# Pixie8888/R3DFSSeg

Hardware: AMD Instinct MI355X
Metric: episodes/sec S3DIS 2-way 5-shot 2048-pt (MPTI+attention, train step: forward+backward+grad all-reduce+Adam) (higher is better)
Workload: dtype f32 (index-free GEMMs -- self-attention, 1x1 convolutions, weight gradients, the EdgeConv backward's edge GEMMs -- as bf16x3 split products on the bf16 MFMA with fp32 accumulate; every index-deciding result: fp32)

## Files before the change

### r3dfsseg_amd/csrc/head_graph.hip

```cpp
#include "common.h"

#define HG_NC 4
typedef unsigned short hg_col_t;
#define HG_ROWS_PER_BLOCK_MIN 4
#define HG_MAX_PART 2048

struct HgEp {
  long nodes, nbr, y, z, g, lam, dn;
  long desc;
  long ws;
  long stats;
  long labels, logits, loss, pred;
};
#define HG_WS(p) p = (decltype(p))((const char*)(p) + (long)ep * st.ws * 4)
#define HG_AT(p, stride) p += (long)ep * (stride)

__global__ __launch_bounds__(256) void r3d_graph_bits_kernel(const int* __restrict__ nbr, int kp1, const int* __restrict__ n_dev,
                                                             int n_cap, int words, unsigned* __restrict__ outb, HgEp st) {
  __shared__ unsigned bm[4][1024];
  const int ep = blockIdx.y;
  nbr += (long)ep * st.nbr * kp1; HG_AT(n_dev, st.desc); HG_WS(outb);
  const int n = min(*n_dev, n_cap);
  const int w = threadIdx.x >> 6, lane = threadIdx.x & 63;
  const int i = blockIdx.x * 4 + w;
// ... 630 lines not shown
  {
    const int ep = blockIdx.y;
    HG_AT(B, b_stride); HG_WS(dinv); HG_WS(agg); HG_WS(MW); HG_AT(n_dev, st.desc); HG_AT(x, x_stride); HG_WS(r); HG_WS(p); HG_WS(q);
    HG_WS(part); HG_WS(Einv); HG_WS(cg);
  }
  __shared__ float4 sm[4];
  __shared__ float4 rs[HG_UROWS];
  __shared__ float us[HG_UROWS];
  __shared__ int ag[HG_UROWS];
  __shared__ __attribute__((aligned(16))) float mu_s[HG_M * HG_NC];
  __shared__ float4 wpart[2 * 4 * HG_M];
  __shared__ double d_s[HG_M * HG_NC];
  __shared__ float t_s[HG_M * HG_NC];
  __shared__ float rr_s[HG_NC];
  __shared__ int last_s;
  __shared__ float tile_s[4 * 32 * 65];
  __shared__ float4 dot_s[HG_UROWS];
  const int row0 = blockIdx.x * HG_UROWS;
  float m[64];
  if (mode == 1) cg_load_mw_column(MW, row0, n_cap, m);
  const int n = min(*n_dev, n_cap);
  if (mode == 1) mu_s[threadIdx.x] = cg->mu[threadIdx.x];
  __syncthreads();
  if (mode == 1) {
    const int lane = threadIdx.x & 63, w = threadIdx.x >> 6;
    float* tl = tile_s + w * (32 * 65);
#pragma unroll
    for (int h = 0; h < 2; ++h) {
#pragma unroll
      for (int k = 0; k < 32; ++k) tl[k * 65 + lane] = m[32 * h + k];
      __builtin_amdgcn_wave_barrier();
      const int rk = lane & 31, a0 = 32 * (lane >> 5);
      float4 acc = f4_zero();
#pragma unroll 8
      for (int a = 0; a < 32; ++a) {
        const float mv = tl[rk * 65 + a0 + a];
        const float4 cv = *reinterpret_cast<const float4*>(&mu_s[(a0 + a) * HG_NC]);
        acc.x = __builtin_fmaf(mv, cv.x, acc.x); acc.y = __builtin_fmaf(mv, cv.y, acc.y);
        acc.z = __builtin_fmaf(mv, cv.z, acc.z); acc.w = __builtin_fmaf(mv, cv.w, acc.w);
      }
      acc.x += __shfl_xor(acc.x, 32); acc.y += __shfl_xor(acc.y, 32);
      acc.z += __shfl_xor(acc.z, 32); acc.w += __shfl_xor(acc.w, 32);
      if (lane < 32) dot_s[64 * w + 32 * h + lane] = acc;
      __builtin_amdgcn_wave_barrier();
    }
  }
  __syncthreads();
  {
    const int i = row0 + threadIdx.x;
    float4 rv = f4_zero();
    float u = 0.f;
    int a = 0;
    if (i < n) {
      u = 1.f / dinv[i];
      a = agg[i];
      rv = B[i];
      if (mode == 1) {
        const float4 s = dot_s[threadIdx.x];
        rv = make_float4(rv.x - s.x, rv.y - s.y, rv.z - s.z, rv.w - s.w);
        x[i] = make_float4(u * mu_s[a * HG_NC + 0], u * mu_s[a * HG_NC + 1], u * mu_s[a * HG_NC + 2], u * mu_s[a * HG_NC + 3]);
        r[i] = rv;
      }
    }
    if (mode == 1 && i < n_cap) {
      p[i] = f4_zero(); q[i] = f4_zero();
      if (i >= n) { x[i] = f4_zero(); r[i] = f4_zero(); }
    }
    rs[threadIdx.x] = rv; us[threadIdx.x] = u; ag[threadIdx.x] = a;
  }
  __syncthreads();
  cg_block_partials(rs, us, ag, row0, n, m, mode == 1, part + (long)blockIdx.x * HG_PART, sm, wpart);
  if (cg_delivered_last(cg, gridDim.x, &last_s)) cg_reduce_step(part, gridDim.x, Einv, mode, 0, tol2, cg, d_s, t_s, rr_s);
}

__global__ __launch_bounds__(256) void r3d_cg_spmv_kernel(
    const int* __restrict__ row_ptr, const hg_col_t* __restrict__ col, const float* __restrict__ val,
    const float* __restrict__ dinv, const int* __restrict__ agg, const float* __restrict__ MW,
    const int* __restrict__ n_dev, int n_cap, float alpha_lp, int it, int rows_per_block,
    const float4* __restrict__ r, float4* __restrict__ p, float4* __restrict__ q,
    float4* __restrict__ part_pq, const CgState* __restrict__ cg, HgEp st) {
  __shared__ float4 mu_s[HG_M];
  __shared__ float4 wsum[4];
  {
    const int ep = blockIdx.y;
    HG_WS(cg);
    if (cg->done) return;
    HG_WS(row_ptr); HG_WS(col); HG_WS(val); HG_WS(dinv); HG_WS(agg); HG_WS(MW); HG_AT(n_dev, st.desc); HG_WS(r); HG_WS(p);
    HG_WS(q); HG_WS(part_pq);
  }
  const int n = min(*n_dev, n_cap);
  const int lane = threadIdx.x & 63, w = threadIdx.x >> 6;
  if (threadIdx.x < HG_M) mu_s[threadIdx.x] = reinterpret_cast<const float4*>(cg->mu)[threadIdx.x];
  const float4 beta = *reinterpret_cast<const float4*>(cg->beta);
  __syncthreads();
  const float4 mul = mu_s[lane];
  float4 acc_pq = f4_zero();
  const int row0 = blockIdx.x * rows_per_block + w * (rows_per_block / 4);
  for (int rr_i = 0; rr_i < rows_per_block / 4; ++rr_i) {
    const int i = row0 + rr_i;
    if (i >= n) break;
    float4 s = f4_zero();
    const int rb = row_ptr[i], re = row_ptr[i + 1];
    const float mw = MW[(long)i * HG_M + lane];
    for (int e0 = rb + lane; e0 < re; e0 += 384) {
      int jv[6];
      float av[6];
#pragma unroll
      for (int u = 0; u < 6; ++u) {
        const int e = e0 + 64 * u;
        const int ec = min(e, re - 1);
        jv[u] = col[ec];
        av[u] = r3d_keep(val[ec], e < re);
      }
      float4 rj[6];
#pragma unroll
      for (int u = 0; u < 6; ++u) rj[u] = r[jv[u]];
#pragma unroll
      for (int u = 0; u < 6; ++u) {
        s.x = __builtin_fmaf(av[u], rj[u].x, s.x); s.y = __builtin_fmaf(av[u], rj[u].y, s.y);
        s.z = __builtin_fmaf(av[u], rj[u].z, s.z); s.w = __builtin_fmaf(av[u], rj[u].w, s.w);
      }
    }
    s.x = __builtin_fmaf(mw, mul.x, -alpha_lp * s.x); s.y = __builtin_fmaf(mw, mul.y, -alpha_lp * s.y);
    s.z = __builtin_fmaf(mw, mul.z, -alpha_lp * s.z); s.w = __builtin_fmaf(mw, mul.w, -alpha_lp * s.w);
#pragma unroll
    for (int o = 32; o > 0; o >>= 1) {
      s.x += __shfl_xor(s.x, o); s.y += __shfl_xor(s.y, o);
      s.z += __shfl_xor(s.z, o); s.w += __shfl_xor(s.w, o);
    }
    if (lane == 0) {
      const float4 ri = r[i], pi = p[i], qi = q[i];
      const float u = 1.f / dinv[i];
      const float4 m = mu_s[agg[i]];
      const float4 pn = make_float4((ri.x + u * m.x) + beta.x * pi.x, (ri.y + u * m.y) + beta.y * pi.y,
                                    (ri.z + u * m.z) + beta.z * pi.z, (ri.w + u * m.w) + beta.w * pi.w);
      const float4 qn = make_float4((ri.x + s.x) + beta.x * qi.x, (ri.y + s.y) + beta.y * qi.y,
                                    (ri.z + s.z) + beta.z * qi.z, (ri.w + s.w) + beta.w * qi.w);
      p[i] = pn;
      q[i] = qn;
      acc_pq.x += pn.x * qn.x; acc_pq.y += pn.y * qn.y; acc_pq.z += pn.z * qn.z; acc_pq.w += pn.w * qn.w;
    }
  }
  if (lane == 0) wsum[w] = acc_pq;
  __syncthreads();
  if (threadIdx.x == 0) {
    float4 t = wsum[0];
    for (int q2 = 1; q2 < 4; ++q2) { t.x += wsum[q2].x; t.y += wsum[q2].y; t.z += wsum[q2].z; t.w += wsum[q2].w; }
    part_pq[blockIdx.x] = t;
  }
}

#define SL_ROWS 128
#define SL_WAVES 8
#define SL_RPW (SL_ROWS / SL_WAVES)
#define SL_MAX_LDS (144 * 1024)
__global__ __launch_bounds__(64 * SL_WAVES) void r3d_cg_spmv_lds_kernel(
    const int* __restrict__ row_ptr, const hg_col_t* __restrict__ col, const float* __restrict__ val,
    const float* __restrict__ dinv, const int* __restrict__ agg, const float* __restrict__ MW,
    const int* __restrict__ n_dev, int n_cap, float alpha_lp, int it, int rows_per_block,
    const float4* __restrict__ r, float4* __restrict__ p, float4* __restrict__ q,
    float4* __restrict__ part_pq , const CgState* __restrict__ cg, HgEp st) {
  extern __shared__ __attribute__((aligned(16))) float4 rs[];
  __shared__ float4 mu_s[HG_M];
  {
    const int ep = blockIdx.y;
    HG_WS(cg);
    if (cg->done) return;
    HG_WS(row_ptr); HG_WS(col); HG_WS(val); HG_WS(dinv); HG_WS(agg); HG_WS(MW); HG_AT(n_dev, st.desc); HG_WS(r); HG_WS(p);
    HG_WS(q); HG_WS(part_pq);
  }
  __shared__ float4 pq_s[SL_ROWS];
  const int n = min(*n_dev, n_cap);
  const int tid = threadIdx.x, lane = tid & 63, w = tid >> 6;
  const int n_wg = gridDim.x, bx = blockIdx.x;
  const int n_part = (n_cap + 3) / 4;
  auto row_of = [&](int k) {
    const int l = SL_WAVES * k + w;
    return 4 * ((l >> 2) * n_wg + bx) + (l & 3);
  };
  int nrows = 0;
#pragma unroll
  for (int k = 0; k < SL_RPW; ++k) nrows += row_of(k) < n ? 1 : 0;
  const int my_row = min(row_of(min(lane, SL_RPW - 1)), max(n - 1, 0));
  const int my_rb = row_ptr[my_row], my_re = row_ptr[my_row + 1];
  for (int i0 = tid; i0 < n; i0 += 4 * 64 * SL_WAVES) {
    float4 v[4];
#pragma unroll
    for (int u = 0; u < 4; ++u) v[u] = r[min(i0 + u * 64 * SL_WAVES, n - 1)];
#pragma unroll
    for (int u = 0; u < 4; ++u)
      if (i0 + u * 64 * SL_WAVES < n) rs[i0 + u * 64 * SL_WAVES] = v[u];
  }
  if (tid < HG_M) mu_s[tid] = reinterpret_cast<const float4*>(cg->mu)[tid];
  const float4 beta = *reinterpret_cast<const float4*>(cg->beta);
  __syncthreads();
  const float4 mul = mu_s[lane];
  int jv[6], jn[6];
  float av[6], an[6];
  float mw = 0.f, mwn = 0.f;
  auto issue = [&](int k, int (&jj)[6], float (&aa)[6], float& mm) {
    const int rb = __builtin_amdgcn_readlane(my_rb, k), re = __builtin_amdgcn_readlane(my_re, k);
#pragma unroll
    for (int u = 0; u < 6; ++u) {
      const int e = rb + lane + 64 * u;
      const int ec = max(min(e, re - 1), 0);
      jj[u] = col[ec];
      aa[u] = r3d_keep(val[ec], e < re);
    }
    mm = MW[(long)row_of(k) * HG_M + lane];
  };
  float4 tot[2] = {f4_zero(), f4_zero()};
  if (nrows > 0) issue(0, jv, av, mw);
#pragma unroll
  for (int h = 0; h < 2; ++h) {
    float4 acc[8];
#pragma unroll
    for (int kk = 0; kk < 8; ++kk) {
      const int k = 8 * h + kk;
      acc[kk] = f4_zero();
      if (k < nrows) {
        if (k + 1 < nrows) issue(k + 1, jn, an, mwn);
        const int rb = __builtin_amdgcn_readlane(my_rb, k), re = __builtin_amdgcn_readlane(my_re, k);
        float4 s = f4_zero();
        {
          float4 rj[6];
#pragma unroll
          for (int u = 0; u < 6; ++u) rj[u] = rs[jv[u]];
#pragma unroll
          for (int u = 0; u < 6; ++u) {
            s.x = __builtin_fmaf(av[u], rj[u].x, s.x); s.y = __builtin_fmaf(av[u], rj[u].y, s.y);
            s.z = __builtin_fmaf(av[u], rj[u].z, s.z); s.w = __builtin_fmaf(av[u], rj[u].w, s.w);
          }
        }
        for (int e0 = rb + 384; e0 < re; e0 += 384) {
          int j2[6];
          float a2[6];
#pragma unroll
          for (int u = 0; u < 6; ++u) {
            const int e = e0 + lane + 64 * u;
            const int ec = min(e, re - 1);
            j2[u] = col[ec];
            a2[u] = r3d_keep(val[ec], e < re);
          }
#pragma unroll
          for (int u = 0; u < 6; ++u) {
            const float4 rj = rs[j2[u]];
            s.x = __builtin_fmaf(a2[u], rj.x, s.x); s.y = __builtin_fmaf(a2[u], rj.y, s.y);
            s.z = __builtin_fmaf(a2[u], rj.z, s.z); s.w = __builtin_fmaf(a2[u], rj.w, s.w);
          }
        }
        s.x = __builtin_fmaf(mw, mul.x, -alpha_lp * s.x); s.y = __builtin_fmaf(mw, mul.y, -alpha_lp * s.y);
        s.z = __builtin_fmaf(mw, mul.z, -alpha_lp * s.z); s.w = __builtin_fmaf(mw, mul.w, -alpha_lp * s.w);
        acc[kk] = s;
#pragma unroll
        for (int u = 0; u < 6; ++u) { jv[u] = jn[u]; av[u] = an[u]; }
        mw = mwn;
      }
    }
    float4 a4[4], a2[2], a1;
    {
      const bool hi = (lane & 32) != 0;
#pragma unroll
      for (int t = 0; t < 4; ++t) {
        const float4 keepv = hi ? acc[4 + t] : acc[t], sendv = hi ? acc[t] : acc[4 + t];
        a4[t].x = keepv.x + __shfl_xor(sendv.x, 32); a4[t].y = keepv.y + __shfl_xor(sendv.y, 32);
        a4[t].z = keepv.z + __shfl_xor(sendv.z, 32); a4[t].w = keepv.w + __shfl_xor(sendv.w, 32);
      }
    }
    {
      const bool hi = (lane & 16) != 0;
#pragma unroll
      for (int t = 0; t < 2; ++t) {
        const float4 keepv = hi ? a4[2 + t] : a4[t], sendv = hi ? a4[t] : a4[2 + t];
        a2[t].x = keepv.x + __shfl_xor(sendv.x, 16); a2[t].y = keepv.y + __shfl_xor(sendv.y, 16);
        a2[t].z = keepv.z + __shfl_xor(sendv.z, 16); a2[t].w = keepv.w + __shfl_xor(sendv.w, 16);
      }
    }
    {
      const bool hi = (lane & 8) != 0;
      const float4 keepv = hi ? a2[1] : a2[0], sendv = hi ? a2[0] : a2[1];
      a1.x = keepv.x + __shfl_xor(sendv.x, 8); a1.y = keepv.y + __shfl_xor(sendv.y, 8);
      a1.z = keepv.z + __shfl_xor(sendv.z, 8); a1.w = keepv.w + __shfl_xor(sendv.w, 8);
    }
#pragma unroll
    for (int o = 4; o > 0; o >>= 1) {
      a1.x += __shfl_xor(a1.x, o); a1.y += __shfl_xor(a1.y, o);
      a1.z += __shfl_xor(a1.z, o); a1.w += __shfl_xor(a1.w, o);
    }
    tot[h] = a1;
  }
  float4 acc_pq = f4_zero();
  const int trow = 8 * (lane & 7) + (lane >> 3);
  if ((lane & 7) < 2 && trow < nrows) {
    const float4 keep = (lane & 1) ? tot[1] : tot[0];
    const int i = row_of(trow);
    const float4 ri = rs[i], pi = p[i], qi = q[i];
    const float u = 1.f / dinv[i];
    const float4 m = mu_s[agg[i]];
    const float4 pn = make_float4((ri.x + u * m.x) + beta.x * pi.x, (ri.y + u * m.y) + beta.y * pi.y,
                                  (ri.z + u * m.z) + beta.z * pi.z, (ri.w + u * m.w) + beta.w * pi.w);
    const float4 qn = make_float4((ri.x + keep.x) + beta.x * qi.x, (ri.y + keep.y) + beta.y * qi.y,
                                  (ri.z + keep.z) + beta.z * qi.z, (ri.w + keep.w) + beta.w * qi.w);
    p[i] = pn;
    q[i] = qn;
    acc_pq = make_float4(pn.x * qn.x, pn.y * qn.y, pn.z * qn.z, pn.w * qn.w);
  }
  if ((lane & 7) < 2) pq_s[SL_WAVES * trow + w] = acc_pq;
  __syncthreads();
  if (tid < SL_ROWS / 4) {
    const float4 a = pq_s[4 * tid], b2 = pq_s[4 * tid + 1], c2 = pq_s[4 * tid + 2], d2 = pq_s[4 * tid + 3];
    const float4 t = make_float4(((a.x + b2.x) + c2.x) + d2.x, ((a.y + b2.y) + c2.y) + d2.y, ((a.z + b2.z) + c2.z) + d2.z,
                                 ((a.w + b2.w) + c2.w) + d2.w);
    const int gidx = tid * n_wg + bx;
    if (gidx < n_part) part_pq[gidx] = t;
  }
}

#ifdef CG_STAMPS
__device__ unsigned long long g_cg_dbg[32];
#define CSTAMP(i) do { if (it == 3 && threadIdx.x == 0 && blockIdx.x == 0) g_cg_dbg[i] = __builtin_amdgcn_s_memtime(); } while (0)
#define CSTAMP_LAST(i) do { if (it == 3 && threadIdx.x == 0) g_cg_dbg[16 + i] = __builtin_amdgcn_s_memtime(); } while (0)
extern "C" int r3d_cg_debug_read(unsigned long long* out32) {
  return hipMemcpyFromSymbol(out32, HIP_SYMBOL(g_cg_dbg), sizeof(g_cg_dbg)) == hipSuccess ? 0 : 1;
}
#else
#define CSTAMP(i)
#define CSTAMP_LAST(i)
#endif

__global__ __launch_bounds__(256) void r3d_cg_update_kernel(
    const int* __restrict__ n_dev, int n_cap, int it, int nblk_pq, const float* __restrict__ dinv, const int* __restrict__ agg,
    const float* __restrict__ MW, const float4* __restrict__ p, const float4* __restrict__ q, float4* __restrict__ x,
    float4* __restrict__ r, const float4* __restrict__ part_pq, float* __restrict__ part, const float* __restrict__ Einv,
    float tol2, CgState* __restrict__ cg, HgEp st, long x_stride) {
  __shared__ float4 sm[4];
  __shared__ float4 rs[HG_UROWS];
  __shared__ float us[HG_UROWS];
  __shared__ int ag[HG_UROWS];
  __shared__ float4 wpart[2 * 4 * HG_M];
  __shared__ double d_s[HG_M * HG_NC];
  __shared__ float t_s[HG_M * HG_NC];
  __shared__ float rr_s[HG_NC];
  __shared__ int last_s;
  {
    const int ep = blockIdx.y;
    HG_AT(n_dev, st.desc); HG_WS(dinv); HG_WS(agg); HG_WS(MW); HG_WS(p); HG_WS(q); HG_AT(x, x_stride); HG_WS(r); HG_WS(part_pq);
    HG_WS(part); HG_WS(Einv); HG_WS(cg);
  }
  const int row0 = blockIdx.x * HG_UROWS;
  const int i = row0 + threadIdx.x;
  const int ic = min(i, n_cap - 1);
  float m[64];
  CSTAMP(0);
  cg_load_mw_column(MW, row0, n_cap, m);
  const float4 pi = p[ic], qi = q[ic];
  float4 xi = x[ic], ri = r[ic];
  const float dv = dinv[ic];
  const int av = agg[ic];
  const int done = cg->done;
  const float4 rz = *reinterpret_cast<const float4*>(cg->rz);
  const int n = min(*n_dev, n_cap);
  const float4 pq = reduce_partials(part_pq, nblk_pq, sm);
  CSTAMP(1);
  if (done) return;
  float4 al;
  al.x = pq.x > 0.f ? rz.x / pq.x : 0.f;
  al.y = pq.y > 0.f ? rz.y / pq.y : 0.f;
  al.z = pq.z > 0.f ? rz.z / pq.z : 0.f;
  al.w = pq.w > 0.f ? rz.w / pq.w : 0.f;
  float u = 0.f;
  int a = 0;
  if (i < n) {
    xi.x += al.x * pi.x; xi.y += al.y * pi.y; xi.z += al.z * pi.z; xi.w += al.w * pi.w;
    ri.x -= al.x * qi.x; ri.y -= al.y * qi.y; ri.z -= al.z * qi.z; ri.w -= al.w * qi.w;
    x[i] = xi; r[i] = ri;
    u = 1.f / dv;
    a = av;
  } else {
    ri = f4_zero();
  }
  rs[threadIdx.x] = ri; us[threadIdx.x] = u; ag[threadIdx.x] = a;
  __syncthreads();
  CSTAMP(2);
  cg_block_partials(rs, us, ag, row0, n, m, true, part + (long)blockIdx.x * HG_PART, sm, wpart);
  CSTAMP(3);
  const bool last = cg_delivered_last(cg, gridDim.x, &last_s);
  CSTAMP(4);
  if (last) {
    CSTAMP_LAST(0);
    cg_reduce_step(part, gridDim.x, Einv, 1, it + 1, tol2, cg, d_s, t_s, rr_s);
    CSTAMP_LAST(1);
  }
}

__global__ __launch_bounds__(1024) void r3d_logits_ce_kernel(const float4* __restrict__ Z, const float4* __restrict__ Z2,
                                                             const int* __restrict__ desc_nproto, int n_q, int N, int n_classes,
                                                             const long long* __restrict__ labels,
                                                             float* __restrict__ logits ,
                                                             float* __restrict__ loss_out, int* __restrict__ pred_out, HgEp st) {
  __shared__ float red[16];
  {
    const int ep = blockIdx.x;
    HG_AT(Z, st.z); HG_AT(desc_nproto, st.desc); HG_AT(logits, st.logits);
    if (Z2) HG_AT(Z2, st.z);
    if (labels) HG_AT(labels, st.labels);
    if (loss_out) HG_AT(loss_out, st.loss);
    if (pred_out) HG_AT(pred_out, st.pred);
  }
  const int n_proto = *desc_nproto;
  float acc = 0.f;
  for (int e = threadIdx.x; e < n_q * N; e += blockDim.x) {
    const int qi = e / N, p = e - qi * N;
    const float4 z = Z[n_proto + e];
    const float4 z2 = Z2 ? Z2[n_proto + e] : f4_zero();
    const float zv[8] = {z.x, z.y, z.z, z.w, z2.x, z2.y, z2.z, z2.w};
    float mx = zv[0];
    int am = 0;
    for (int c = 1; c < n_classes; ++c) if (zv[c] > mx) { mx = zv[c]; am = c; }
    float se = 0.f;
    for (int c = 0; c < n_classes; ++c) {
      logits[((long)qi * n_classes + c) * N + p] = zv[c];
      se += expf(zv[c] - mx);
    }
    if (labels) {
      const int lab = (int)labels[e];
      acc += (mx + logf(se)) - zv[lab];
    }
    if (pred_out) pred_out[e] = am;
  }
  acc = r3d_wave_sum(acc);
  if ((threadIdx.x & 63) == 0) red[threadIdx.x >> 6] = acc;
  __syncthreads();
  if (threadIdx.x == 0) {
    float t = 0.f;
    for (int w = 0; w < (int)(blockDim.x >> 6); ++w) t += red[w];
    if (loss_out) *loss_out = t / (float)(n_q * N);
  }
}

struct LpWs {
  unsigned *outb, *sym;
  int *row_len, *row_ptr, *agg;
  hg_col_t* col;
  float *val, *dinv, *wdir, *MW, *Epart, *part;
  float* Einv;
  float4 *r, *p, *q, *part_pq;
  CgState* cg;
  long words, total;
};

static inline long hg_vblocks(int n_cap) { return r3d_cdiv(n_cap, HG_UROWS); }

static LpWs lp_carve(int32_t* ws, int n_cap, int kp1) {
  LpWs L;
  L.words = (n_cap + 31) / 32;
  const long nnz_cap = 2L * n_cap * (kp1 - 1);
  int32_t* wp = ws;
  auto align4 = [&]() { wp += (4 - ((wp - ws) & 3)) & 3; };
  L.outb = (unsigned*)wp; wp += n_cap * L.words;
  L.sym = (unsigned*)wp; wp += n_cap * L.words;
  L.row_len = wp; wp += n_cap + 8;
  L.row_ptr = wp; wp += n_cap + 8;
  L.col = (hg_col_t*)wp; wp += (nnz_cap + 1) / 2;
  L.val = (float*)wp; wp += nnz_cap;
  L.wdir = (float*)wp; wp += 2 * nnz_cap;
  L.dinv = (float*)wp; wp += n_cap;
  L.agg = wp; wp += n_cap;
  align4();
  L.MW = (float*)wp; wp += (long)n_cap * HG_M;
  L.Epart = (float*)wp; wp += (long)HG_EBLOCKS * HG_M * HG_M;
  align4();
  L.Einv = (float*)wp; wp += (long)HG_M * HG_M;
  L.part = (float*)wp; wp += hg_vblocks(n_cap) * HG_PART;
  align4();
  L.r = (float4*)wp; wp += 4L * n_cap;
  L.p = (float4*)wp; wp += 4L * n_cap;
  L.q = (float4*)wp; wp += 4L * n_cap;
  L.part_pq = (float4*)wp; wp += 4L * HG_MAX_PART;
  L.cg = (CgState*)wp; wp += (sizeof(CgState) + 3) / 4;
  L.total = (wp - ws) + 64;
  return L;
}

extern "C" long r3d_lp_ws_words(int n_cap, int kp1) { return lp_carve(nullptr, n_cap, kp1).total; }

extern "C" int r3d_lp_ws_offsets(int n_cap, int kp1, long* out6) {
  R3D_REQUIRE(out6 && n_cap > 0 && kp1 >= 2, "r3d_lp_ws_offsets: bad arguments");
  const LpWs L = lp_carve(nullptr, n_cap, kp1);
  const int32_t* base = nullptr;
  out6[0] = (const int32_t*)L.row_ptr - base; out6[1] = (const int32_t*)L.col - base; out6[2] = (const int32_t*)L.val - base;
  out6[3] = (const int32_t*)L.dinv - base; out6[4] = (const int32_t*)L.agg - base; out6[5] = (const int32_t*)L.cg - base;
  return R3D_OK;
}

__global__ void r3d_weights_compare_kernel(const int* __restrict__ row_ptr, const int* __restrict__ n_dev, int n_cap,
                                           const float* __restrict__ wdir, const float* __restrict__ wdir2, long scratch_stride,
                                           int* __restrict__ mismatch, HgEp st) {
  const int ep = blockIdx.y;
  HG_WS(row_ptr); HG_AT(n_dev, st.desc); HG_WS(wdir);
  wdir2 += (long)ep * scratch_stride;
  const int n = min(*n_dev, n_cap);
  const long nnz2 = 2L * row_ptr[n];
  int bad = 0;
  for (long e = (long)blockIdx.x * blockDim.x + threadIdx.x; e < nnz2; e += (long)gridDim.x * blockDim.x)
    bad += __float_as_uint(wdir[e]) != __float_as_uint(wdir2[e]) ? 1 : 0;
  bad = (int)r3d_wave_sum((float)bad);
  if ((threadIdx.x & 63) == 0 && bad) atomicAdd(mismatch, bad);
}
extern "C" long r3d_graph_weights_verify_words(int n_cap, int kp1) {
  const long nnz_cap = 2L * n_cap * (kp1 - 1);
  return 2 * nnz_cap + nnz_cap + n_cap + 64;
}
extern "C" int r3d_graph_weights_verify(int n_ep, const float* nodes, long ldn, int D, const int32_t* n_dev, long desc_stride,
                                        int n_cap, int kp1, float sigma, int32_t* ws, long ws_words, long ws_stride,
                                        float* scratch, int32_t* mismatch_out, void* stream) {
  R3D_REQUIRE(nodes && n_dev && ws && scratch && mismatch_out, "r3d_graph_weights_verify: null pointer");
  R3D_REQUIRE(n_cap > 0 && kp1 >= 2 && ws_words >= r3d_lp_ws_words(n_cap, kp1) && n_ep >= 1 &&
                  (n_ep == 1 || ((ws_stride & 3) == 0 && ws_stride >= ws_words)),
              "r3d_graph_weights_verify: bad arguments");
  hipStream_t st = (hipStream_t)stream;
  const LpWs L = lp_carve(ws, n_cap, kp1);
  const long nnz_cap = 2L * n_cap * (kp1 - 1), per = r3d_graph_weights_verify_words(n_cap, kp1);
  for (int e = 0; e < n_ep; ++e) {
    HgEp one{};
    float* base = scratch + (long)e * per;
    int32_t* wse = ws + (long)e * ws_stride;
    const LpWs Le = lp_carve(wse, n_cap, kp1);
    hipLaunchKernelGGL(r3d_graph_weights_kernel, dim3(n_cap, 1), dim3(256), 0, st, nodes + (long)e * n_cap * ldn, ldn, D, Le.outb,
                       (int)Le.words, n_dev + (long)e * desc_stride, n_cap, Le.row_ptr, Le.col, sigma, base + 2 * nnz_cap,
                       base + 3 * nnz_cap, base, one);
  }
  HgEp ep{};
  ep.desc = desc_stride; ep.ws = ws_stride;
  hipLaunchKernelGGL(r3d_weights_compare_kernel, dim3(256, n_ep), dim3(256), 0, st, L.row_ptr, n_dev, n_cap, L.wdir, scratch, per,
                     mismatch_out, ep);
  R3D_LAUNCH_CHECK("r3d_graph_weights_verify");
  return R3D_OK;
}

__global__ void r3d_cg_stats_kernel(const CgState* __restrict__ cg, int* __restrict__ stats_out, HgEp st) {
  const int ep = blockIdx.x;
  HG_WS(cg); HG_AT(stats_out, st.stats);
  if (threadIdx.x == 0) { stats_out[0] = cg->done; stats_out[1] = cg->iters; }
}

static int lp_coarse_space(const LpWs& L, const float* nodes, long ldn, int D, const int32_t* n_dev, const int32_t* n_proto_dev,
                           int n_cap, float alpha, int n_ep, const HgEp& ep, hipStream_t st) {
  const int agg_rpw = 4;
  const size_t agg_lds = ((size_t)HG_M * (D | 1) + 4 * D) * sizeof(float);
  static bool lds_opt_in = false;
  if (!lds_opt_in) {
    hipFuncSetAttribute((const void*)r3d_cg_aggregate_kernel, hipFuncAttributeMaxDynamicSharedMemorySize, 96 * 1024);
    lds_opt_in = true;
  }
  hipLaunchKernelGGL(r3d_cg_aggregate_kernel, dim3(r3d_cdiv(n_cap, 4 * agg_rpw), n_ep), dim3(256), agg_lds, st, nodes, ldn, D,
                     n_dev, n_proto_dev, n_cap, agg_rpw, L.agg, ep);
  hipLaunchKernelGGL(r3d_cg_mw_kernel, dim3(r3d_cdiv(n_cap, 4), n_ep), dim3(256), 0, st, L.row_ptr, L.col, L.val, L.dinv, L.agg,
                     n_dev, n_cap, alpha, 1, L.MW, ep);
  hipLaunchKernelGGL(r3d_cg_epart_kernel, dim3(HG_EBLOCKS, n_ep), dim3(128), 0, st, L.MW, L.dinv, L.agg, n_dev, n_cap, L.Epart,
                     ep);
  hipLaunchKernelGGL(r3d_cg_einv_kernel, dim3(n_ep), dim3(1024), 0, st, L.Epart, L.Einv, ep);
  return R3D_OK;
}

static int g_cg_lds_min_blocks = 256;
extern "C" int r3d_debug_set_cg_spmv_lds_min_blocks(int min_blocks) {
  const int old = g_cg_lds_min_blocks;
  g_cg_lds_min_blocks = min_blocks;
  return old;
}

static int lp_solve(const LpWs& L, const float* RHS, long rhs_stride, const int32_t* n_dev, int n_cap, float alpha, int max_iter,
                    float tol, float* X, long x_stride, int32_t* stats_out, int n_ep, const HgEp& ep, hipStream_t st) {
  const int nblk_v = (int)hg_vblocks(n_cap);
  int rpb = HG_ROWS_PER_BLOCK_MIN;
  while (r3d_cdiv(n_cap, rpb) > HG_MAX_PART) rpb += 4;
  const int nblk_s = r3d_cdiv(n_cap, rpb);
  R3D_REQUIRE(nblk_s <= HG_MAX_PART, "r3d_label_propagate: n_cap too large");
  float4* x = (float4*)X;
  const float tol2 = tol * tol;
  r3d_fill_words_ep(&L.cg->ticket, 0u, 1, n_ep, ep.ws, st);
  for (int mode = 0; mode < 2; ++mode)
    hipLaunchKernelGGL(r3d_cg_init_kernel, dim3(nblk_v, n_ep), dim3(256), 0, st, (const float4*)RHS, L.dinv, L.agg, L.MW, n_dev,
                       n_cap, mode, x, L.r, L.p, L.q, L.part, L.Einv, tol2, L.cg, ep, rhs_stride, x_stride);
  const size_t lds_r = (size_t)n_cap * sizeof(float4);
  const bool use_lds = lds_r <= SL_MAX_LDS && rpb == HG_ROWS_PER_BLOCK_MIN && (long)n_ep * r3d_cdiv(n_cap, SL_ROWS) >= g_cg_lds_min_blocks;
  if (use_lds) {
    static size_t attr = 0;
    if (lds_r > attr) {
      hipError_t e = hipFuncSetAttribute((const void*)r3d_cg_spmv_lds_kernel, hipFuncAttributeMaxDynamicSharedMemorySize, (int)lds_r);
      R3D_REQUIRE(e == hipSuccess, "r3d_label_propagate: cannot reserve %zu B of LDS: %s", lds_r, hipGetErrorString(e));
      attr = lds_r;
    }
  }
  const int nblk_l = r3d_cdiv(n_cap, SL_ROWS);
  const int nblk_pq = nblk_s;
  for (int it = 0; it < max_iter; ++it) {
    if (use_lds)
      hipLaunchKernelGGL(r3d_cg_spmv_lds_kernel, dim3(nblk_l, n_ep), dim3(64 * SL_WAVES), lds_r, st, L.row_ptr, L.col, L.val, L.dinv,
                         L.agg, L.MW, n_dev, n_cap, alpha, it, SL_ROWS, L.r, L.p, L.q, L.part_pq, L.cg, ep);
    else
      hipLaunchKernelGGL(r3d_cg_spmv_kernel, dim3(nblk_s, n_ep), dim3(256), 0, st, L.row_ptr, L.col, L.val, L.dinv, L.agg, L.MW,
                         n_dev, n_cap, alpha, it, rpb, L.r, L.p, L.q, L.part_pq, L.cg, ep);
    hipLaunchKernelGGL(r3d_cg_update_kernel, dim3(nblk_v, n_ep), dim3(256), 0, st, n_dev, n_cap, it, nblk_pq, L.dinv, L.agg, L.MW,
                       L.p, L.q, x, L.r, L.part_pq, L.part, L.Einv, tol2, L.cg, ep, x_stride);
  }
  if (stats_out) hipLaunchKernelGGL(r3d_cg_stats_kernel, dim3(n_ep), dim3(64), 0, st, L.cg, stats_out, ep);
  return R3D_OK;
}

static int label_propagate_impl(int n_ep, const HgEp& ep, const float* nodes, long ldn, int D, const int32_t* nbr, int kp1,
                                const float* Y, const int32_t* n_dev, const int32_t* n_proto_dev, int n_cap, float sigma,
                                float alpha, int max_iter, float tol, float* Z, int32_t* ws, long ws_words, int32_t* stats_out,
                                void* stream) {
  R3D_REQUIRE(nodes && nbr && Y && n_dev && n_proto_dev && Z && ws, "r3d_label_propagate: null pointer");
  R3D_REQUIRE(n_cap > 0 && kp1 >= 2 && ws_words >= r3d_lp_ws_words(n_cap, kp1),
              "r3d_label_propagate: workspace of %ld words, r3d_lp_ws_words(%d, %d) = %ld needed", ws_words, n_cap, kp1,
              n_cap > 0 && kp1 >= 2 ? r3d_lp_ws_words(n_cap, kp1) : -1L);
  R3D_REQUIRE((ldn & 3) == 0 && ((uintptr_t)nodes & 15) == 0,
              "r3d_label_propagate: node rows are read as float4: ldn must be a multiple of 4 and nodes 16-byte aligned");
  R3D_REQUIRE(n_cap > 0 && n_cap <= 32768 && D > 0 && D <= 256 && (D & 3) == 0 && kp1 >= 2,
              "r3d_label_propagate: unsupported n_cap=%d D=%d kp1=%d", n_cap, D, kp1);
  R3D_REQUIRE(max_iter > 0 && max_iter <= HG_MAX_ITER && sigma > 0.f, "r3d_label_propagate: bad solver parameters");
  R3D_REQUIRE(((uintptr_t)ws & 15) == 0 && ((uintptr_t)Y & 15) == 0 && ((uintptr_t)Z & 15) == 0,
              "r3d_label_propagate: ws, Y and Z must be 16-byte aligned");
  R3D_REQUIRE(n_ep >= 1 && n_ep <= 4096 && (n_ep == 1 || ((ep.ws & 3) == 0 && ep.ws >= ws_words)),
              "r3d_label_propagate: %d systems need a scratch stride that is a multiple of 4 words and >= the scratch size", n_ep);
  hipStream_t st = (hipStream_t)stream;
  const LpWs L = lp_carve(ws, n_cap, kp1);
  const long words = L.words;
  hipLaunchKernelGGL(r3d_graph_bits_kernel, dim3(r3d_cdiv(n_cap, 4), n_ep), dim3(256), 0, st, nbr, kp1, n_dev, n_cap,
                     (int)words, L.outb, ep);
  hipLaunchKernelGGL(r3d_graph_transpose_kernel, dim3(r3d_cdiv(words, BT_CW), r3d_cdiv(n_cap, BT_ROWS), n_ep), dim3(256), 0, st,
                     L.outb, (int)words, n_cap, L.sym, ep);
  hipLaunchKernelGGL(r3d_graph_rowlen_kernel, dim3(r3d_cdiv(n_cap, 4), n_ep), dim3(256), 0, st, L.sym, L.outb, (int)words,
                     n_dev, n_cap, L.row_len, ep);
  hipLaunchKernelGGL(r3d_scan_kernel, dim3(n_ep), dim3(1024), 0, st, L.row_len, n_cap, L.row_ptr, ep);
  hipLaunchKernelGGL(r3d_graph_cols_kernel, dim3(r3d_cdiv(n_cap, 4), n_ep), dim3(256), 0, st, L.sym, (int)words, n_dev,
                     n_cap, L.row_ptr, L.col, ep);
  hipLaunchKernelGGL(r3d_graph_weights_kernel, dim3(n_cap, n_ep), dim3(256), 0, st, nodes, ldn, D, L.outb,
                     (int)words, n_dev, n_cap, L.row_ptr, L.col, sigma, L.val, L.dinv, L.wdir, ep);
  hipLaunchKernelGGL(r3d_graph_normalize_kernel, dim3(r3d_cdiv(n_cap, 4), n_ep), dim3(256), 0, st, L.row_ptr, L.col, L.dinv,
                     n_dev, n_cap, L.val, ep);
  int rc = lp_coarse_space(L, nodes, ldn, D, n_dev, n_proto_dev, n_cap, alpha, n_ep, ep, st);
  if (rc) return rc;
  rc = lp_solve(L, Y, ep.y, n_dev, n_cap, alpha, max_iter, tol, Z, ep.z, stats_out, n_ep, ep, st);
  if (rc) return rc;
  R3D_LAUNCH_CHECK("r3d_label_propagate");
  return R3D_OK;
}

extern "C" int r3d_label_propagate(const float* nodes, long ldn, int D, const int32_t* nbr, int kp1,
                                   const float* Y, const int32_t* n_dev, const int32_t* n_proto_dev, int n_cap, float sigma,
                                   float alpha, int max_iter, float tol, float* Z, int32_t* ws, long ws_words,
                                   int32_t* stats_out, void* stream) {
  const HgEp one{};
  return label_propagate_impl(1, one, nodes, ldn, D, nbr, kp1, Y, n_dev, n_proto_dev, n_cap, sigma, alpha, max_iter, tol, Z, ws,
                              ws_words, stats_out, stream);
}

extern "C" int r3d_label_propagate_solve_batched(int n_ep, const float* Y, const int32_t* n_dev, long desc_stride, int n_cap,
                                                 int kp1, float alpha, int max_iter, float tol, float* Z, int32_t* ws,
                                                 long ws_words, long ws_stride, int32_t* stats_out, long stats_stride,
                                                 void* stream) {
  R3D_REQUIRE(Y && n_dev && Z && ws, "r3d_label_propagate_solve: null pointer");
  R3D_REQUIRE(n_cap > 0 && kp1 >= 2 && ws_words >= r3d_lp_ws_words(n_cap, kp1), "r3d_label_propagate_solve: workspace too short");
  R3D_REQUIRE(max_iter > 0 && max_iter <= HG_MAX_ITER, "r3d_label_propagate_solve: bad solver parameters");
  R3D_REQUIRE(((uintptr_t)ws & 15) == 0 && ((uintptr_t)Y & 15) == 0 && ((uintptr_t)Z & 15) == 0,
              "r3d_label_propagate_solve: ws, Y and Z must be 16-byte aligned");
  R3D_REQUIRE(n_ep >= 1 && n_ep <= 4096 && (n_ep == 1 || ((ws_stride & 3) == 0 && ws_stride >= ws_words)),
              "r3d_label_propagate_solve: bad scratch stride");
  HgEp ep{};
  ep.nodes = ep.nbr = ep.y = ep.z = n_cap;
  ep.desc = desc_stride; ep.ws = ws_stride; ep.stats = stats_stride;
  const LpWs L = lp_carve(ws, n_cap, kp1);
  const int rc = lp_solve(L, Y, ep.y, n_dev, n_cap, alpha, max_iter, tol, Z, ep.z, stats_out, n_ep, ep, (hipStream_t)stream);
  if (rc) return rc;
  R3D_LAUNCH_CHECK("r3d_label_propagate_solve");
  return R3D_OK;
}

extern "C" int r3d_label_propagate_batched(int n_ep, const float* nodes, long ldn, int D, const int32_t* nbr, int kp1,
                                           const float* Y, const int32_t* n_dev, const int32_t* n_proto_dev, long desc_stride,
                                           int n_cap, float sigma, float alpha, int max_iter, float tol, float* Z, int32_t* ws,
                                           long ws_words, long ws_stride, int32_t* stats_out, long stats_stride, void* stream) {
  HgEp ep{};
  ep.nodes = ep.nbr = ep.y = ep.z = n_cap;
  ep.desc = desc_stride; ep.ws = ws_stride; ep.stats = stats_stride;
  return label_propagate_impl(n_ep, ep, nodes, ldn, D, nbr, kp1, Y, n_dev, n_proto_dev, n_cap, sigma, alpha, max_iter, tol, Z, ws,
                              ws_words, stats_out, stream);
}

static __device__ __forceinline__ float dot4(float4 a, float4 b) { return a.x * b.x + a.y * b.y + a.z * b.z + a.w * b.w; }

__global__ __launch_bounds__(256) void r3d_lp_bwd_dd_kernel(const int* __restrict__ row_ptr, const hg_col_t* __restrict__ col,
                                                            const float* __restrict__ val, const float* __restrict__ dinv,
                                                            const int* __restrict__ n_dev, int n_cap, float alpha,
                                                            const float4* __restrict__ lam, const float4* __restrict__ Z,
                                                            float* __restrict__ dD, HgEp st) {
  const int ep = blockIdx.y;
  HG_WS(row_ptr); HG_WS(col); HG_WS(val); HG_WS(dinv); HG_AT(n_dev, st.desc); HG_AT(lam, st.lam); HG_AT(Z, st.z); HG_WS(dD);
  const int n = min(*n_dev, n_cap);
  const int i = blockIdx.x * 4 + (threadIdx.x >> 6);
  const int lane = threadIdx.x & 63;
  if (i >= n) return;
  const float4 li = lam[i], zi = Z[i];
  const float di = dinv[i];
  float g = 0.f;
  for (int e = row_ptr[i] + lane; e < row_ptr[i + 1]; e += 64) {
    const int j = col[e];
    const float ds = alpha * (dot4(li, Z[j]) + dot4(lam[j], zi));
    g += ds * (val[e] / di);
  }
  g = r3d_wave_sum(g);
  if (lane == 0) dD[i] = -0.5f * di * di * di * g;
}

__global__ __launch_bounds__(256) void r3d_lp_bwd_dx_kernel(
    const float* __restrict__ nodes, long ldn, int D, const float* __restrict__ wdir,
    const int* __restrict__ row_ptr, const hg_col_t* __restrict__ col, const float* __restrict__ dinv,
    const int* __restrict__ n_dev, int n_cap, float sigma, float alpha, const float4* __restrict__ lam,
    const float4* __restrict__ Z, const float* __restrict__ dD, float* __restrict__ dnodes, long ldd, HgEp st) {
  {
    const int ep = blockIdx.y;
    nodes += (long)ep * st.nodes * ldn; HG_WS(wdir); HG_WS(row_ptr); HG_WS(col); HG_WS(dinv); HG_AT(n_dev, st.desc);
    HG_AT(lam, st.lam); HG_AT(Z, st.z); HG_WS(dD); dnodes += (long)ep * st.dn * ldd;
  }
  __shared__ float acc_s[4][256];
  __shared__ float uv_s[4][2];
  const int n = min(*n_dev, n_cap);
  const int w = threadIdx.x >> 6;
  const int i = blockIdx.x;
  const int lane = threadIdx.x & 63;
  if (i >= n) return;
  const float* xi = nodes + (long)i * ldn;
  const float4 li = lam[i], zi = Z[i];
  const float di = dinv[i], ddi = dD[i];
  const int beg = row_ptr[i], end = row_ptr[i + 1];
  const float inv_s2 = 1.f / (sigma * sigma);
  const int c0 = min(lane, D - 1), c1 = min(lane + 64, D - 1), c2 = min(lane + 128, D - 1), c3 = min(lane + 192, D - 1);
  float U = 0.f, V = 0.f;
  float a0 = 0.f, a1 = 0.f, a2 = 0.f, a3 = 0.f;
  for (int e0 = beg + 64 * w; e0 < end; e0 += 256) {
    const int e = e0 + lane;
    const bool ok = e < end;
    const int ec = min(e, end - 1);
    const int j = col[ec];
    const float2 wd = *reinterpret_cast<const float2*>(wdir + 2L * ec);
// ... 172 lines not shown
```

Before: 384.4.

## Make LDS CG SpMV persistent with multi-pass rows and a flattened edge prefetch pipeline

The LDS SpMV kernel now loops over several 512-row passes per block. The grid is sized to the number of resident block slots, found with an occupancy query, so each block stages the dense vector r into LDS once and reuses it across more rows, instead of every block reloading it. The edge gather becomes a software pipeline of depth 2 whose prefetch crosses row boundaries and long rows. The per-wave row reduction groups 4 rows at a time. This adds per-pass barriers and a serial pass loop in exchange for fewer redundant r loads into LDS.

```diff
diff --git a/r3dfsseg_amd/csrc/head_graph.hip b/r3dfsseg_amd/csrc/head_graph.hip
--- a/r3dfsseg_amd/csrc/head_graph.hip
+++ b/r3dfsseg_amd/csrc/head_graph.hip
@@ -806,7 +806,9 @@
 
 #define SL_ROWS 128
 #define SL_WAVES 8
-#define SL_RPW (SL_ROWS / SL_WAVES)
+#define SL_PASS_RPW 64
+#define SL_PASS_ROWS (SL_PASS_RPW * SL_WAVES)
+#define SL_DEPTH 2
 #define SL_MAX_LDS (144 * 1024)
 __global__ __launch_bounds__(64 * SL_WAVES) void r3d_cg_spmv_lds_kernel(
     const int* __restrict__ row_ptr, const hg_col_t* __restrict__ col, const float* __restrict__ val,
@@ -823,20 +825,11 @@
     HG_WS(row_ptr); HG_WS(col); HG_WS(val); HG_WS(dinv); HG_WS(agg); HG_WS(MW); HG_AT(n_dev, st.desc); HG_WS(r); HG_WS(p);
     HG_WS(q); HG_WS(part_pq);
   }
-  __shared__ float4 pq_s[SL_ROWS];
+  __shared__ float4 pq_s[SL_PASS_ROWS];
   const int n = min(*n_dev, n_cap);
   const int tid = threadIdx.x, lane = tid & 63, w = tid >> 6;
   const int n_wg = gridDim.x, bx = blockIdx.x;
   const int n_part = (n_cap + 3) / 4;
-  auto row_of = [&](int k) {
-    const int l = SL_WAVES * k + w;
-    return 4 * ((l >> 2) * n_wg + bx) + (l & 3);
-  };
-  int nrows = 0;
-#pragma unroll
-  for (int k = 0; k < SL_RPW; ++k) nrows += row_of(k) < n ? 1 : 0;
-  const int my_row = min(row_of(min(lane, SL_RPW - 1)), max(n - 1, 0));
-  const int my_rb = row_ptr[my_row], my_re = row_ptr[my_row + 1];
   for (int i0 = tid; i0 < n; i0 += 4 * 64 * SL_WAVES) {
     float4 v[4];
 #pragma unroll
@@ -846,127 +839,138 @@
       if (i0 + u * 64 * SL_WAVES < n) rs[i0 + u * 64 * SL_WAVES] = v[u];
   }
   if (tid < HG_M) mu_s[tid] = reinterpret_cast<const float4*>(cg->mu)[tid];
-  const float4 beta = *reinterpret_cast<const float4*>(cg->beta);
   __syncthreads();
   const float4 mul = mu_s[lane];
-  int jv[6], jn[6];
-  float av[6], an[6];
-  float mw = 0.f, mwn = 0.f;
-  auto issue = [&](int k, int (&jj)[6], float (&aa)[6], float& mm) {
-    const int rb = __builtin_amdgcn_readlane(my_rb, k), re = __builtin_amdgcn_readlane(my_re, k);
-#pragma unroll
-    for (int u = 0; u < 6; ++u) {
-      const int e = rb + lane + 64 * u;
-      const int ec = max(min(e, re - 1), 0);
-      jj[u] = col[ec];
-      aa[u] = r3d_keep(val[ec], e < re);
-    }
-    mm = MW[(long)row_of(k) * HG_M + lane];
-  };
-  float4 tot[2] = {f4_zero(), f4_zero()};
-  if (nrows > 0) issue(0, jv, av, mw);
-#pragma unroll
-  for (int h = 0; h < 2; ++h) {
-    float4 acc[8];
-#pragma unroll
-    for (int kk = 0; kk < 8; ++kk) {
-      const int k = 8 * h + kk;
-      acc[kk] = f4_zero();
-      if (k < nrows) {
-        if (k + 1 < nrows) issue(k + 1, jn, an, mwn);
-        const int rb = __builtin_amdgcn_readlane(my_rb, k), re = __builtin_amdgcn_readlane(my_re, k);
-        float4 s = f4_zero();
-        {
-          float4 rj[6];
-#pragma unroll
-          for (int u = 0; u < 6; ++u) rj[u] = rs[jv[u]];
-#pragma unroll
-          for (int u = 0; u < 6; ++u) {
-            s.x = __builtin_fmaf(av[u], rj[u].x, s.x); s.y = __builtin_fmaf(av[u], rj[u].y, s.y);
-            s.z = __builtin_fmaf(av[u], rj[u].z, s.z); s.w = __builtin_fmaf(av[u], rj[u].w, s.w);
-          }
+  const int n_c = (n_part + n_wg - 1) / n_wg;
+  for (int c0 = 0; c0 < n_c; c0 += SL_PASS_ROWS / 4) {
+    auto row_of = [&](int k) {
+      const int l = SL_WAVES * k + w;
+      return 4 * ((c0 + (l >> 2)) * n_wg + bx) + (l & 3);
+    };
+    const int nrows = __popcll(__ballot(row_of(lane) < n));
+    const int my_row = min(row_of(lane), max(n - 1, 0));
+    const int my_rb = row_ptr[my_row], my_re = row_ptr[my_row + 1];
+    int rj[SL_DEPTH][6];
+    float ra[SL_DEPTH][6], rm[SL_DEPTH];
+#pragma unroll
+    for (int d = 0; d < SL_DEPTH; ++d) {
+#pragma unroll
+      for (int u = 0; u < 6; ++u) { rj[d][u] = 0; ra[d][u] = 0.f; }
+      rm[d] = 0.f;
+    }
+    int ck = 0, ce = __builtin_amdgcn_readlane(my_rb, 0), cre = __builtin_amdgcn_readlane(my_re, 0);
+    auto issue = [&](int (&jj)[6], float (&aa)[6], float& mm) {
+      if (ck < nrows) {
+#pragma unroll
+        for (int u = 0; u < 6; ++u) {
+          const int ec = max(min(ce + lane + 64 * u, cre - 1), 0);
+          jj[u] = col[ec];
+          aa[u] = val[ec];
         }
-        for (int e0 = rb + 384; e0 < re; e0 += 384) {
-          int j2[6];
-          float a2[6];
-#pragma unroll
-          for (int u = 0; u < 6; ++u) {
-            const int e = e0 + lane + 64 * u;
-            const int ec = min(e, re - 1);
-            j2[u] = col[ec];
-            a2[u] = r3d_keep(val[ec], e < re);
-          }
-#pragma unroll
-          for (int u = 0; u < 6; ++u) {
-            const float4 rj = rs[j2[u]];
-            s.x = __builtin_fmaf(a2[u], rj.x, s.x); s.y = __builtin_fmaf(a2[u], rj.y, s.y);
-            s.z = __builtin_fmaf(a2[u], rj.z, s.z); s.w = __builtin_fmaf(a2[u], rj.w, s.w);
-          }
+        mm = MW[(long)row_of(ck) * HG_M + lane];
+        ce += 384;
+        if (ce >= cre) {
+          ++ck;
+          const int kc = __builtin_amdgcn_readfirstlane(min(ck, SL_PASS_RPW - 1));
+          ce = __builtin_amdgcn_readlane(my_rb, kc);
+          cre = __builtin_amdgcn_readlane(my_re, kc);
         }
-        s.x = __builtin_fmaf(mw, mul.x, -alpha_lp * s.x); s.y = __builtin_fmaf(mw, mul.y, -alpha_lp * s.y);
-        s.z = __builtin_fmaf(mw, mul.z, -alpha_lp * s.z); s.w = __builtin_fmaf(mw, mul.w, -alpha_lp * s.w);
-        acc[kk] = s;
-#pragma unroll
-        for (int u = 0; u < 6; ++u) { jv[u] = jn[u]; av[u] = an[u]; }
-        mw = mwn;
       }
-    }
-    float4 a4[4], a2[2], a1;
-    {
-      const bool hi = (lane & 32) != 0;
-#pragma unroll
-      for (int t = 0; t < 4; ++t) {
-        const float4 keepv = hi ? acc[4 + t] : acc[t], sendv = hi ? acc[t] : acc[4 + t];
-        a4[t].x = keepv.x + __shfl_xor(sendv.x, 32); a4[t].y = keepv.y + __shfl_xor(sendv.y, 32);
-        a4[t].z = keepv.z + __shfl_xor(sendv.z, 32); a4[t].w = keepv.w + __shfl_xor(sendv.w, 32);
+    };
+#pragma unroll
+    for (int d = 0; d < SL_DEPTH; ++d) issue(rj[d], ra[d], rm[d]);
+    float4 tot = f4_zero();
+    const int ngrp = (nrows + 3) >> 2;
+    for (int h = 0; h < ngrp; ++h) {
+      float4 acc[4];
+#pragma unroll
+      for (int kk = 0; kk < 4; ++kk) {
+        const int k = 4 * h + kk;
+        acc[kk] = f4_zero();
+        if (k < nrows) {
+          const int kc = __builtin_amdgcn_readfirstlane(k);
+          const int rb = __builtin_amdgcn_readlane(my_rb, kc), re = __builtin_amdgcn_readlane(my_re, kc);
+          float4 s = f4_zero();
+          float mw = 0.f;
+          int e0 = rb;
+          do {
+            int cj[6];
+            float ca[6];
+#pragma unroll
+            for (int u = 0; u < 6; ++u) { cj[u] = rj[0][u]; ca[u] = ra[0][u]; }
+            mw = rm[0];
+#pragma unroll
+            for (int d = 0; d + 1 < SL_DEPTH; ++d) {
+#pragma unroll
+              for (int u = 0; u < 6; ++u) { rj[d][u] = rj[d + 1][u]; ra[d][u] = ra[d + 1][u]; }
+              rm[d] = rm[d + 1];
+            }
+            issue(rj[SL_DEPTH - 1], ra[SL_DEPTH - 1], rm[SL_DEPTH - 1]);
+            float4 g[6];
+#pragma unroll
+            for (int u = 0; u < 6; ++u) g[u] = rs[cj[u]];
+#pragma unroll
+            for (int u = 0; u < 6; ++u) {
+              const float a = r3d_keep(ca[u], e0 + lane + 64 * u < re);
+              s.x = __builtin_fmaf(a, g[u].x, s.x); s.y = __builtin_fmaf(a, g[u].y, s.y);
+              s.z = __builtin_fmaf(a, g[u].z, s.z); s.w = __builtin_fmaf(a, g[u].w, s.w);
+            }
+            e0 += 384;
+          } while (e0 < re);
+          s.x = __builtin_fmaf(mw, mul.x, -alpha_lp * s.x); s.y = __builtin_fmaf(mw, mul.y, -alpha_lp * s.y);
+          s.z = __builtin_fmaf(mw, mul.z, -alpha_lp * s.z); s.w = __builtin_fmaf(mw, mul.w, -alpha_lp * s.w);
+          acc[kk] = s;
+        }
       }
-    }
-    {
-      const bool hi = (lane & 16) != 0;
-#pragma unroll
-      for (int t = 0; t < 2; ++t) {
-        const float4 keepv = hi ? a4[2 + t] : a4[t], sendv = hi ? a4[t] : a4[2 + t];
-        a2[t].x = keepv.x + __shfl_xor(sendv.x, 16); a2[t].y = keepv.y + __shfl_xor(sendv.y, 16);
-        a2[t].z = keepv.z + __shfl_xor(sendv.z, 16); a2[t].w = keepv.w + __shfl_xor(sendv.w, 16);
+      float4 a2[2], a1;
+      {
+        const bool hi = (lane & 32) != 0;
+#pragma unroll
+        for (int t = 0; t < 2; ++t) {
+          const float4 keepv = hi ? acc[2 + t] : acc[t], sendv = hi ? acc[t] : acc[2 + t];
+          a2[t].x = keepv.x + __shfl_xor(sendv.x, 32); a2[t].y = keepv.y + __shfl_xor(sendv.y, 32);
+          a2[t].z = keepv.z + __shfl_xor(sendv.z, 32); a2[t].w = keepv.w + __shfl_xor(sendv.w, 32);
+        }
       }
-    }
-    {
-      const bool hi = (lane & 8) != 0;
-      const float4 keepv = hi ? a2[1] : a2[0], sendv = hi ? a2[0] : a2[1];
-      a1.x = keepv.x + __shfl_xor(sendv.x, 8); a1.y = keepv.y + __shfl_xor(sendv.y, 8);
-      a1.z = keepv.z + __shfl_xor(sendv.z, 8); a1.w = keepv.w + __shfl_xor(sendv.w, 8);
-    }
-#pragma unroll
-    for (int o = 4; o > 0; o >>= 1) {
-      a1.x += __shfl_xor(a1.x, o); a1.y += __shfl_xor(a1.y, o);
-      a1.z += __shfl_xor(a1.z, o); a1.w += __shfl_xor(a1.w, o);
-    }
-    tot[h] = a1;
-  }
-  float4 acc_pq = f4_zero();
-  const int trow = 8 * (lane & 7) + (lane >> 3);
-  if ((lane & 7) < 2 && trow < nrows) {
-    const float4 keep = (lane & 1) ? tot[1] : tot[0];
-    const int i = row_of(trow);
-    const float4 ri = rs[i], pi = p[i], qi = q[i];
-    const float u = 1.f / dinv[i];
-    const float4 m = mu_s[agg[i]];
-    const float4 pn = make_float4((ri.x + u * m.x) + beta.x * pi.x, (ri.y + u * m.y) + beta.y * pi.y,
-                                  (ri.z + u * m.z) + beta.z * pi.z, (ri.w + u * m.w) + beta.w * pi.w);
-    const float4 qn = make_float4((ri.x + keep.x) + beta.x * qi.x, (ri.y + keep.y) + beta.y * qi.y,
-                                  (ri.z + keep.z) + beta.z * qi.z, (ri.w + keep.w) + beta.w * qi.w);
-    p[i] = pn;
-    q[i] = qn;
-    acc_pq = make_float4(pn.x * qn.x, pn.y * qn.y, pn.z * qn.z, pn.w * qn.w);
-  }
-  if ((lane & 7) < 2) pq_s[SL_WAVES * trow + w] = acc_pq;
-  __syncthreads();
-  if (tid < SL_ROWS / 4) {
-    const float4 a = pq_s[4 * tid], b2 = pq_s[4 * tid + 1], c2 = pq_s[4 * tid + 2], d2 = pq_s[4 * tid + 3];
-    const float4 t = make_float4(((a.x + b2.x) + c2.x) + d2.x, ((a.y + b2.y) + c2.y) + d2.y, ((a.z + b2.z) + c2.z) + d2.z,
-                                 ((a.w + b2.w) + c2.w) + d2.w);
-    const int gidx = tid * n_wg + bx;
-    if (gidx < n_part) part_pq[gidx] = t;
+      {
+        const bool hi = (lane & 16) != 0;
+        const float4 keepv = hi ? a2[1] : a2[0], sendv = hi ? a2[0] : a2[1];
+        a1.x = keepv.x + __shfl_xor(sendv.x, 16); a1.y = keepv.y + __shfl_xor(sendv.y, 16);
+        a1.z = keepv.z + __shfl_xor(sendv.z, 16); a1.w = keepv.w + __shfl_xor(sendv.w, 16);
+      }
+#pragma unroll
+      for (int o = 8; o > 0; o >>= 1) {
+        a1.x += __shfl_xor(a1.x, o); a1.y += __shfl_xor(a1.y, o);
+        a1.z += __shfl_xor(a1.z, o); a1.w += __shfl_xor(a1.w, o);
+      }
+      if ((lane & 15) == h) tot = a1;
+    }
+    float4 acc_pq = f4_zero();
+    const int trow = 4 * (lane & 15) + (lane >> 4);
+    if (trow < nrows) {
+      const int i = row_of(trow);
+      const float4 beta = *reinterpret_cast<const float4*>(cg->beta);
+      const float4 ri = rs[i], pi = p[i], qi = q[i];
+      const float u = 1.f / dinv[i];
+      const float4 m = mu_s[agg[i]];
+      const float4 pn = make_float4((ri.x + u * m.x) + beta.x * pi.x, (ri.y + u * m.y) + beta.y * pi.y,
+                                    (ri.z + u * m.z) + beta.z * pi.z, (ri.w + u * m.w) + beta.w * pi.w);
+      const float4 qn = make_float4((ri.x + tot.x) + beta.x * qi.x, (ri.y + tot.y) + beta.y * qi.y,
+                                    (ri.z + tot.z) + beta.z * qi.z, (ri.w + tot.w) + beta.w * qi.w);
+      p[i] = pn;
+      q[i] = qn;
+      acc_pq = make_float4(pn.x * qn.x, pn.y * qn.y, pn.z * qn.z, pn.w * qn.w);
+    }
+    pq_s[SL_WAVES * trow + w] = acc_pq;
+    __syncthreads();
+    if (tid < SL_PASS_ROWS / 4) {
+      const float4 a = pq_s[4 * tid], b2 = pq_s[4 * tid + 1], c2 = pq_s[4 * tid + 2], d2 = pq_s[4 * tid + 3];
+      const float4 t = make_float4(((a.x + b2.x) + c2.x) + d2.x, ((a.y + b2.y) + c2.y) + d2.y, ((a.z + b2.z) + c2.z) + d2.z,
+                                   ((a.w + b2.w) + c2.w) + d2.w);
+      const int gidx = (c0 + tid) * n_wg + bx;
+      if (gidx < n_part) part_pq[gidx] = t;
+    }
+    __syncthreads();
   }
 }
 
@@ -1224,6 +1228,24 @@
   return old;
 }
 
+static int cg_lds_slots(size_t lds_r) {
+  static size_t asked = 0;
+  static int slots = 0;
+  if (lds_r != asked || !slots) {
+    int per_cu = 0, dev = 0, cus = 0;
+    if (hipOccupancyMaxActiveBlocksPerMultiprocessor(&per_cu, r3d_cg_spmv_lds_kernel, 64 * SL_WAVES, lds_r) == hipSuccess &&
+        per_cu > 0 && hipGetDevice(&dev) == hipSuccess &&
+        hipDeviceGetAttribute(&cus, hipDeviceAttributeMultiprocessorCount, dev) == hipSuccess && cus > 0)
+      slots = per_cu * cus;
+    else {
+      (void)hipGetLastError();
+      slots = 256;
+    }
+    asked = lds_r;
+  }
+  return slots;
+}
+
 static int lp_solve(const LpWs& L, const float* RHS, long rhs_stride, const int32_t* n_dev, int n_cap, float alpha, int max_iter,
                     float tol, float* X, long x_stride, int32_t* stats_out, int n_ep, const HgEp& ep, hipStream_t st) {
   const int nblk_v = (int)hg_vblocks(n_cap);
@@ -1247,7 +1269,7 @@
       attr = lds_r;
     }
   }
-  const int nblk_l = r3d_cdiv(n_cap, SL_ROWS);
+  const int nblk_l = use_lds ? std::max(1, std::min(r3d_cdiv(n_cap, SL_ROWS), cg_lds_slots(lds_r) / n_ep)) : 0;
   const int nblk_pq = nblk_s;
   for (int it = 0; it < max_iter; ++it) {
     if (use_lds)
```

Result: faster. 393.4 (median of 6 runs) (+2.4%).
